# TheShadow29/VidSitu

Hardware: AMD Instinct MI355X
Metric: clips/s (10s@32x224x224) SlowFast+TxEnc fwd+bwd (higher is better)
Workload: dtype bf16

## Files before the change

### vidsitu_amd/csrc/conv_wgrad.hip

```cpp
#include <stdlib.h>

#include "common.h"

#include <mutex>
#include <type_traits>
#include "glue_bodies.h"

typedef __attribute__((ext_vector_type(4))) short s16x4;
typedef __attribute__((address_space(3))) s16x4 lds_s16x4;

struct WgradP {
  const uint16_t* dy;
  const uint16_t* x;
  float* out;
  int P;
  int Cout, Kp, Cin, x_ld, dy_ld;
  int To, Ho, Wo, Ti, Hi, Wi;
  int kT, kH, kW, sT, sH, sW, pT, pH, pW;
  int tilesM, tilesN, S, rows_per_split;
  unsigned x_bytes, dy_bytes;
  int xcd_order;
  int dbg;
  const float* in_scale;
  const float* in_shift;
};

#define WG_OOB 0x80000000u

#define WG_ROWTAB 1024

__device__ __forceinline__ int wg_swz_chunk(int row) {
  return ((row & 3) << 1) | (((row >> 3) & 1) << 3);
}

template <int BM, int BN, int WM, int WN, int MODE>
__global__ __launch_bounds__(256) void conv_wgrad_kernel(WgradP p) {
  extern __shared__ __attribute__((aligned(16))) char smem[];
  constexpr int TM = BM / WM, TN = BN / WN;
  constexpr int MR = TM / 16, NR = TN / 16;
  constexpr int CM = BM / 8, CN = BN / 8;
  constexpr int RPM = 256 / CM, RPN = 256 / CN;
  constexpr int IM = (64 + RPM - 1) / RPM, IN = (64 + RPN - 1) / RPN;
  constexpr int IMG = 64 * 256;
  constexpr int STAGE = 2 * IMG;
  static_assert(WM * WN == 4, "4 waves");

  const int tid = threadIdx.x;
  int bid = blockIdx.x;
  if (p.xcd_order) {
    const int nwg = gridDim.x, q = nwg >> 3, r = nwg & 7, xcd = blockIdx.x & 7;
    bid = (xcd < r ? xcd * (q + 1) : r * (q + 1) + (xcd - r) * q) + (blockIdx.x >> 3);
  }
  const int ntile = p.tilesM * p.tilesN;
  const int s = bid / ntile;
  bid -= s * ntile;
  const int tn = bid % p.tilesN, tm = bid / p.tilesN;
  const int m0 = tm * BM, n0 = tn * BN;
  const int pbeg = s * p.rows_per_split;
  const int pend = min(p.P, pbeg + p.rows_per_split);

  int4* rowtab = (int4*)(smem + 2 * STAGE);

  const int ccm = tid % CM, rm = tid / CM;
  const int ccn = tid % CN, rn = tid / CN;
  const bool mcol_ok = (m0 + ccm * 8) < p.Cout;
  const int ncol = n0 + ccn * 8;
  const bool ncol_ok = ncol < p.Kp;
  int dt = 0, dh = 0, dw = 0, c0 = 0;
  if (MODE == 1 && ncol_ok) {
    const int tap = ncol / p.Cin;
    c0 = ncol - tap * p.Cin;
    dw = tap % p.kW;
    const int t2 = tap / p.kW;
    dh = t2 % p.kH;
    dt = t2 / p.kH;
  }

  u32x4 ra[IM], rb[IN];
  const __amdgpu_buffer_rsrc_t xsrc =
      __builtin_amdgcn_make_buffer_rsrc((void*)p.x, 0, (int)p.x_bytes, 0x00020000);
  const __amdgpu_buffer_rsrc_t dysrc =
      __builtin_amdgcn_make_buffer_rsrc((void*)p.dy, 0, (int)p.dy_bytes, 0x00020000);
  const unsigned dycol = (unsigned)((m0 + ccm * 8) * 2);
  const unsigned xtap = (MODE == 1)
      ? (unsigned)(((((long long)dt * p.Hi + dh) * p.Wi + dw) * p.x_ld + c0) * 2)
      : (unsigned)(ncol * 2);

  auto gload = [&](int pstep, int chunk0) __attribute__((always_inline)) {
#pragma unroll
    for (int i = 0; i < IM; ++i) {
      const int r = rm + RPM * i;
      const int pp = pstep + r;
      const unsigned ok = (unsigned)(r < 64) & (unsigned)mcol_ok & (unsigned)(pp < pend);
      const unsigned off = ok ? (unsigned)pp * (unsigned)(p.dy_ld * 2) + dycol : WG_OOB;
      ra[i] = __builtin_bit_cast(u32x4, __builtin_amdgcn_raw_buffer_load_b128(dysrc, off, 0, 0));
    }
#pragma unroll
    for (int i = 0; i < IN; ++i) {
      const int r = rn + RPN * i;
      const int pp = pstep + r;
      unsigned ok = (unsigned)(r < 64) & (unsigned)ncol_ok & (unsigned)(pp < pend);
      unsigned off;
      if (MODE == 0) {
        off = (unsigned)pp * (unsigned)(p.x_ld * 2) + xtap;
      } else {
        const int4 e = rowtab[(pp - chunk0) & (WG_ROWTAB - 1)];
        const int ti = e.y + dt, hi = e.z + dh, wi = e.w + dw;
        ok &= (unsigned)((unsigned)ti < (unsigned)p.Ti) & (unsigned)((unsigned)hi < (unsigned)p.Hi) &
              (unsigned)((unsigned)wi < (unsigned)p.Wi);
        off = (unsigned)e.x + xtap;
      }
      rb[i] = __builtin_bit_cast(u32x4, __builtin_amdgcn_raw_buffer_load_b128(xsrc, ok ? off : WG_OOB, 0, 0));
    }
  };

  auto sstore = [&](int buf) __attribute__((always_inline)) {
    char* A = smem + buf * STAGE;
    char* B = A + IMG;
#pragma unroll
    for (int i = 0; i < IM; ++i) {
      const int r = rm + RPM * i;
      if (r < 64) *(u32x4*)(A + r * 256 + ((ccm ^ wg_swz_chunk(r)) << 4)) = ra[i];
    }
#pragma unroll
    for (int i = 0; i < IN; ++i) {
      const int r = rn + RPN * i;
      if (r < 64) *(u32x4*)(B + r * 256 + ((ccn ^ wg_swz_chunk(r)) << 4)) = rb[i];
    }
  };

  const int wave = tid >> 6, lane = tid & 63;
  const int wm = wave / WN, wn = wave % WN;
  const int g = lane >> 4, li = lane & 15, q = li >> 2, pp4 = li & 3;

  f32x4 acc[MR][NR];
#pragma unroll
  for (int a = 0; a < MR; ++a)
#pragma unroll
    for (int b = 0; b < NR; ++b) acc[a][b] = (f32x4){0.f, 0.f, 0.f, 0.f};

  auto compute = [&](int buf) __attribute__((always_inline)) {
    const char* A = smem + buf * STAGE;
    const char* B = A + IMG;
#pragma unroll
    for (int ks = 0; ks < 2; ++ks) {
      const int row = ks * 32 + 8 * g + q;
      const int swz = ((row & 3) << 2) | (((row >> 3) & 1) << 4);
      bf16x8 af[MR], bfr[NR];
#pragma unroll
      for (int a = 0; a < MR; ++a) {
        const int unit = ((wm * TM + a * 16) >> 2) + pp4;
        const lds_s16x4* ptr = (const lds_s16x4*)(A + row * 256 + ((unit ^ swz) << 3));
        const s16x4 lo = __builtin_amdgcn_ds_read_tr16_b64_v4i16((lds_s16x4*)ptr);
        const s16x4 hi = __builtin_amdgcn_ds_read_tr16_b64_v4i16((lds_s16x4*)(ptr + 128));
        typedef __attribute__((ext_vector_type(8))) short s16x8;
        const s16x8 v = __builtin_shufflevector(lo, hi, 0, 1, 2, 3, 4, 5, 6, 7);
        af[a] = __builtin_bit_cast(bf16x8, v);
      }
#pragma unroll
      for (int b = 0; b < NR; ++b) {
        const int unit = ((wn * TN + b * 16) >> 2) + pp4;
        const lds_s16x4* ptr = (const lds_s16x4*)(B + row * 256 + ((unit ^ swz) << 3));
        const s16x4 lo = __builtin_amdgcn_ds_read_tr16_b64_v4i16((lds_s16x4*)ptr);
        const s16x4 hi = __builtin_amdgcn_ds_read_tr16_b64_v4i16((lds_s16x4*)(ptr + 128));
        typedef __attribute__((ext_vector_type(8))) short s16x8;
        const s16x8 v = __builtin_shufflevector(lo, hi, 0, 1, 2, 3, 4, 5, 6, 7);
        bfr[b] = __builtin_bit_cast(bf16x8, v);
      }
#pragma unroll
      for (int a = 0; a < MR; ++a)
#pragma unroll
        for (int b = 0; b < NR; ++b)
          acc[a][b] = __builtin_amdgcn_mfma_f32_16x16x32_bf16(af[a], bfr[b], acc[a][b], 0, 0, 0);
    }
  };

  for (int chunk0 = pbeg; chunk0 < pend; chunk0 += WG_ROWTAB) {
    const int cend = min(pend, chunk0 + WG_ROWTAB);
    if (MODE == 1) {
      __syncthreads();
      for (int i = tid; i < WG_ROWTAB; i += 256) {
        const int pp = chunk0 + i;
        int4 e = make_int4(0, -(1 << 20), -(1 << 20), -(1 << 20));
        if (pp < cend) {
          int wo, t1, ho, t2, to, n;
          if (p.P < (1 << 24)) {
            fast_divmod(pp, p.Wo, 1.0f / (float)p.Wo, t1, wo);
            fast_divmod(t1, p.Ho, 1.0f / (float)p.Ho, t2, ho);
            fast_divmod(t2, p.To, 1.0f / (float)p.To, n, to);
          } else {
            wo = pp % p.Wo; t1 = pp / p.Wo;
            ho = t1 % p.Ho; t2 = t1 / p.Ho;
            to = t2 % p.To; n = t2 / p.To;
          }
          e.y = to * p.sT - p.pT;
          e.z = ho * p.sH - p.pH;
          e.w = wo * p.sW - p.pW;
          const long long pos0 = (((long long)n * p.Ti + e.y) * p.Hi + e.z) * p.Wi + e.w;
          e.x = (int)(unsigned)(pos0 * p.x_ld * 2);
        }
        rowtab[i] = e;
      }
      __syncthreads();
    }
    const int nsteps = (cend - chunk0 + 63) >> 6;
    gload(chunk0, chunk0);
    __syncthreads();
    sstore(0);
    __syncthreads();
    for (int st = 0; st < nsteps - 1; ++st) {
      const int cur = st & 1;
      gload(chunk0 + (st + 1) * 64, chunk0);
      __builtin_amdgcn_sched_barrier(0);
      compute(cur);
      __builtin_amdgcn_sched_barrier(0);
      sstore(cur ^ 1);
      __syncthreads();
    }
    compute((nsteps - 1) & 1);
    __syncthreads();
  }

  float* dst = p.out + (long long)s * p.Cout * p.Kp;
#pragma unroll
  for (int a = 0; a < MR; ++a)
#pragma unroll
    for (int b = 0; b < NR; ++b) {
      const int col = n0 + wn * TN + b * 16 + li;
#pragma unroll
      for (int r = 0; r < 4; ++r) {
        const int row = m0 + wm * TM + a * 16 + g * 4 + r;
        if (row < p.Cout && col < p.Kp) dst[(long long)row * p.Kp + col] = acc[a][b][r];
      }
    }
}

template <int BM, int BN, int WM, int WN, int MODE, int NS, bool AOL = false, int ROWS = 64>
__device__ __forceinline__ void conv_wgrad_ring_body(const WgradP& p, const int blk, const int nblk) {
  static_assert(!AOL || MODE == 0, "apply on load: pointwise launches");
  static_assert(ROWS == 64, "stage depth (the half-depth variant of round 4 was measured slower and removed)");
  extern __shared__ __attribute__((aligned(16))) char smem[];
  constexpr int TM = BM / WM, TN = BN / WN;
  constexpr int MR = TM / 16, NR = TN / 16;
  constexpr int CM = BM / 8, CN = BN / 8;
  constexpr int IMG = ROWS * 256;
  constexpr int STAGE = 2 * IMG;
  constexpr int D = NS - 1;
  constexpr int RG = ROWS / 16;
  constexpr int L = 2 * RG;
  constexpr int SPC = WG_ROWTAB / ROWS;
  static_assert(WM * WN == 4, "4 waves");
  static_assert((D - 1) * L <= 63, "vmcnt range");

  const int tid = threadIdx.x;
  int bid = blk;
  if (p.xcd_order) {
    const int nwg = nblk, q = nwg >> 3, r = nwg & 7, xcd = blk & 7;
    bid = (xcd < r ? xcd * (q + 1) : r * (q + 1) + (xcd - r) * q) + (blk >> 3);
  }
  const int ntile = p.tilesM * p.tilesN;
  const int s = bid / ntile;
  bid -= s * ntile;
  const int tn = bid % p.tilesN, tm = bid / p.tilesN;
  const int m0 = tm * BM, n0 = tn * BN;
  const int pbeg = s * p.rows_per_split;
  const int pend = min(p.P, pbeg + p.rows_per_split);
  const int nsteps = (pend - pbeg + ROWS - 1) / ROWS;
  int2* rowtab = (int2*)(smem + NS * STAGE);

  const int wv = __builtin_amdgcn_readfirstlane(tid >> 6), lane = tid & 63;
  const int rg = lane >> 4, cc = lane & 15;
  const int lc = cc ^ ((rg << 1) | ((wv >> 1) << 3));
  const bool mcol_ok = lc < CM && (m0 + lc * 8) < p.Cout;
  const int ncol = n0 + lc * 8;
  const bool ncol_ok = lc < CN && ncol < p.Kp;
  int tap = 0, c0 = 0, dt = 0, dh = 0, dw = 0;
  if (MODE == 1 && ncol_ok) {
    tap = ncol / p.Cin;
    c0 = ncol - tap * p.Cin;
    dw = tap % p.kW;
    const int t2 = tap / p.kW;
    dh = t2 % p.kH;
    dt = t2 / p.kH;
  }
  const unsigned dycol = (unsigned)((m0 + lc * 8) * 2);
  const unsigned xtap = (MODE == 1)
      ? (unsigned)(((((long long)dt * p.Hi + dh) * p.Wi + dw) * p.x_ld + c0) * 2)
      : (unsigned)(ncol * 2);
  const unsigned dy_pitch = (unsigned)(p.dy_ld * 2), x_pitch = (unsigned)(p.x_ld * 2);

  typedef __attribute__((address_space(3))) char* lds_ptr_t;
  const unsigned lds0 = (unsigned)(unsigned long)(lds_ptr_t)smem + (unsigned)wv * 1024u;
  auto rsrc_words = [](const void* base, unsigned bytes) __attribute__((always_inline)) {
    const unsigned long a = (unsigned long)base;
    return (i32x4){(int)(unsigned)a, (int)((unsigned)(a >> 32) & 0xffffu), (int)bytes, 0x00020000};
  };
  const i32x4 xdesc = rsrc_words(p.x, p.x_bytes), dydesc = rsrc_words(p.dy, p.dy_bytes);
  auto dma16 = [](const i32x4& desc, unsigned lds_addr, unsigned voff) __attribute__((always_inline)) {
    asm volatile("s_mov_b32 m0, %0\n\ts_nop 0\n\tbuffer_load_dwordx4 %1, %2, 0 offen lds"
                 :
                 : "s"(lds_addr), "v"(voff), "s"(desc)
                 : "memory");
  };

  const bool small_p = p.P < (1 << 24);
  const float rcpWo = 1.0f / (float)p.Wo, rcpHo = 1.0f / (float)p.Ho, rcpTo = 1.0f / (float)p.To;
  auto build_tab = [&](int chunk) __attribute__((always_inline)) {
    int2* tab = rowtab + (chunk & 1) * WG_ROWTAB;
    const int base = pbeg + chunk * WG_ROWTAB;
    for (int i = tid; i < WG_ROWTAB; i += 256) {
      const int pp = base + i;
      int2 e = make_int2(0, 0);
      if (pp < pend) {
        int wo, t1, ho, t2, to, n;
        if (small_p) {
          fast_divmod(pp, p.Wo, rcpWo, t1, wo);
          fast_divmod(t1, p.Ho, rcpHo, t2, ho);
          fast_divmod(t2, p.To, rcpTo, n, to);
        } else {
          wo = pp % p.Wo; t1 = pp / p.Wo;
          ho = t1 % p.Ho; t2 = t1 / p.Ho;
          to = t2 % p.To; n = t2 / p.To;
        }
        const int ti0 = to * p.sT - p.pT, hi0 = ho * p.sH - p.pH, wi0 = wo * p.sW - p.pW;
        const long long pos0 = (((long long)n * p.Ti + ti0) * p.Hi + hi0) * p.Wi + wi0;
        e.x = (int)(unsigned)(pos0 * p.x_ld * 2);
        unsigned mt = 0u, mh = 0u, mw = 0u;
        for (int a = 0; a < p.kT; ++a) mt |= ((unsigned)(ti0 + a) < (unsigned)p.Ti ? 1u : 0u) << a;
        for (int a = 0; a < p.kH; ++a) mh |= ((unsigned)(hi0 + a) < (unsigned)p.Hi ? 1u : 0u) << a;
        for (int a = 0; a < p.kW; ++a) mw |= ((unsigned)(wi0 + a) < (unsigned)p.Wi ? 1u : 0u) << a;
        unsigned mk = 0u;
        int tp = 0;
        for (int a = 0; a < p.kT; ++a)
          for (int b = 0; b < p.kH; ++b) {
            const unsigned th = (mt >> a) & (mh >> b) & 1u;
            mk |= (th ? mw : 0u) << tp;
            tp += p.kW;
          }
        e.y = (int)mk;
      }
      tab[i] = e;
    }
  };

  auto dma = [&](int st, int stage) __attribute__((always_inline)) {
    const unsigned A = lds0 + (unsigned)(stage * STAGE);
    const unsigned B = A + IMG;
    const int rel0 = st * ROWS + 4 * wv + rg;
    int2 ent[RG];
    if (MODE == 1) {
#pragma unroll
      for (int i = 0; i < RG; ++i) {
        const int rel = rel0 + 16 * i;
        ent[i] = rowtab[((rel >> 10) & 1) * WG_ROWTAB + (rel & (WG_ROWTAB - 1))];
      }
    }
#pragma unroll
    for (int i = 0; i < RG; ++i) {
      const int rel = rel0 + 16 * i;
      const int pp = pbeg + rel;
      const unsigned ok = (unsigned)mcol_ok & (unsigned)(pp < pend);
      dma16(dydesc, A + i * 4096, ok ? (unsigned)pp * dy_pitch + dycol : WG_OOB);
    }
#pragma unroll
    for (int i = 0; i < RG; ++i) {
      const int rel = rel0 + 16 * i;
      const int pp = pbeg + rel;
      unsigned ok = (unsigned)ncol_ok & (unsigned)(pp < pend);
      unsigned off;
      if (MODE == 0) {
        off = (unsigned)pp * x_pitch + xtap;
      } else {
        ok &= ((unsigned)ent[i].y >> tap) & 1u;
        off = (unsigned)ent[i].x + xtap;
      }
      dma16(xdesc, B + i * 4096, ok ? off : WG_OOB);
    }
  };

  const int wm = wv / WN, wn = wv % WN;
  const int g = lane >> 4, li = lane & 15, q = li >> 2, pp4 = li & 3;
  f32x4 acc[MR][NR];
#pragma unroll
  for (int a = 0; a < MR; ++a)
#pragma unroll
    for (int b = 0; b < NR; ++b) acc[a][b] = (f32x4){0.f, 0.f, 0.f, 0.f};

  float asc[NR], ash[NR];
#pragma unroll
  for (int b = 0; b < NR; ++b) {
    const int col = n0 + wn * TN + b * 16 + li;
    asc[b] = (AOL && col < p.Kp) ? p.in_scale[col] : 0.f;
    ash[b] = (AOL && col < p.Kp) ? p.in_shift[col] : 0.f;
  }
  auto compute = [&](int stage) __attribute__((always_inline)) {
    const char* A = smem + stage * STAGE;
    const char* B = A + IMG;
#pragma unroll
    for (int ks = 0; ks < ROWS / 32; ++ks) {
      const int row = ks * 32 + 8 * g + q;
      const int swz = ((row & 3) << 2) | (((row >> 3) & 1) << 4);
      bf16x8 af[MR], bfr[NR];
      typedef __attribute__((ext_vector_type(8))) short s16x8;
#pragma unroll
      for (int a = 0; a < MR; ++a) {
        const int unit = ((wm * TM + a * 16) >> 2) + pp4;
        const lds_s16x4* ptr = (const lds_s16x4*)(A + row * 256 + ((unit ^ swz) << 3));
        const s16x4 lo = __builtin_amdgcn_ds_read_tr16_b64_v4i16((lds_s16x4*)ptr);
        const s16x4 hi = __builtin_amdgcn_ds_read_tr16_b64_v4i16((lds_s16x4*)(ptr + 128));
        af[a] = __builtin_bit_cast(bf16x8, (s16x8)__builtin_shufflevector(lo, hi, 0, 1, 2, 3, 4, 5, 6, 7));
      }
#pragma unroll
      for (int b = 0; b < NR; ++b) {
        const int unit = ((wn * TN + b * 16) >> 2) + pp4;
        const lds_s16x4* ptr = (const lds_s16x4*)(B + row * 256 + ((unit ^ swz) << 3));
        const s16x4 lo = __builtin_amdgcn_ds_read_tr16_b64_v4i16((lds_s16x4*)ptr);
        const s16x4 hi = __builtin_amdgcn_ds_read_tr16_b64_v4i16((lds_s16x4*)(ptr + 128));
        bfr[b] = __builtin_bit_cast(bf16x8, (s16x8)__builtin_shufflevector(lo, hi, 0, 1, 2, 3, 4, 5, 6, 7));
        if (AOL) bfr[b] = aol_frag_n(bfr[b], asc[b], ash[b]);
      }
#pragma unroll
      for (int a = 0; a < MR; ++a)
#pragma unroll
        for (int b = 0; b < NR; ++b)
          acc[a][b] = __builtin_amdgcn_mfma_f32_16x16x32_bf16(af[a], bfr[b], acc[a][b], 0, 0, 0);
    }
  };

  if (MODE == 1) {
    build_tab(0);
    __syncthreads();
  }
#pragma unroll
  for (int d = 0; d < D; ++d) dma(d, d);
  int st_c = 0, st_l = D;
  for (int st = 0; st < nsteps; ++st) {
    if (!(p.dbg & 4)) asm volatile("s_waitcnt vmcnt(%0) lgkmcnt(0)" ::"i"((D - 1) * L) : "memory");
    if (!(p.dbg & 8)) __builtin_amdgcn_s_barrier();
    __builtin_amdgcn_sched_barrier(0);
    if (MODE == 1 && (st % SPC) == 0 && pbeg + (st / SPC + 1) * WG_ROWTAB < pend && !(p.dbg & 32))
      build_tab(st / SPC + 1);
    if (!(p.dbg & 2)) dma(st + D, st_l);
    __builtin_amdgcn_sched_barrier(0);
    if (!(p.dbg & 1)) compute(st_c);
    __builtin_amdgcn_sched_barrier(0);
    st_c = (st_c + 1 == NS) ? 0 : st_c + 1;
    st_l = (st_l + 1 == NS) ? 0 : st_l + 1;
  }
  asm volatile("s_waitcnt vmcnt(0)" ::: "memory");
  if ((p.dbg & 64) && acc[0][0][0] != 123.456f) return;

  float* dst = p.out + (long long)s * p.Cout * p.Kp;
#pragma unroll
  for (int a = 0; a < MR; ++a)
#pragma unroll
    for (int b = 0; b < NR; ++b) {
      const int col = n0 + wn * TN + b * 16 + li;
#pragma unroll
      for (int r = 0; r < 4; ++r) {
        const int row = m0 + wm * TM + a * 16 + g * 4 + r;
        if (row < p.Cout && col < p.Kp) dst[(long long)row * p.Kp + col] = acc[a][b][r];
      }
    }
}

template <int BM, int BN, int WM, int WN, int MODE, int NS, bool AOL = false, int ROWS = 64>
__global__ __launch_bounds__(256) void conv_wgrad_ring_kernel(WgradP p) {
  conv_wgrad_ring_body<BM, BN, WM, WN, MODE, NS, AOL, ROWS>(p, blockIdx.x, gridDim.x);
}

#define WGD_UNIT (3 * 8192)
#define WGD_NU 6
#define WGD_TAB 512
#define WGD_EP 260

template <int MODE, bool STAG>
__device__ __forceinline__ void conv_wgrad_deep_body(const WgradP& p, const int blk, const int nblk) {
  extern __shared__ __attribute__((aligned(16))) char smem[];
  const int tid = threadIdx.x;
  const int wv = __builtin_amdgcn_readfirstlane(tid >> 6), lane = tid & 63;
  const int hf = wv >> 2, wq = wv & 3;
  int bid = blk;
  if (p.xcd_order) {
    const int nwg = nblk, q = nwg >> 3, r = nwg & 7, xcd = blk & 7;
    bid = (xcd < r ? xcd * (q + 1) : r * (q + 1) + (xcd - r) * q) + (blk >> 3);
  }
  const int ntile = p.tilesM * p.tilesN;
  const int s = bid / ntile;
  bid -= s * ntile;
  const int tn = bid % p.tilesN, tm = bid / p.tilesN;
  const int m0 = tm * 128, n0 = tn * 256;
  const int pbeg = s * p.rows_per_split;
  const int pend = min(p.P, pbeg + p.rows_per_split);
  const int nu = (pend - pbeg + 31) >> 5;
  int2* rowtab = (int2*)(smem + WGD_NU * WGD_UNIT);

  const int rg = lane >> 4, cc = lane & 15;
  const int lc = cc ^ ((rg << 1) | (((STAG ? wv : wq) >> 1 & 1) << 3));
  const bool mcol_ok = (m0 + lc * 8) < p.Cout;
  const unsigned dycol = (unsigned)((m0 + lc * 8) * 2);
  bool ncol_ok[2];
  int tap[2];
  unsigned xtap[2];
#pragma unroll
  for (int i = 0; i < 2; ++i) {
    const int ncol = n0 + i * 128 + lc * 8;
    ncol_ok[i] = ncol < p.Kp;
    tap[i] = 0;
    xtap[i] = (unsigned)(ncol * 2);
    if (MODE == 1 && ncol_ok[i]) {
      tap[i] = ncol / p.Cin;
      const int c0 = ncol - tap[i] * p.Cin;
      const int dw = tap[i] % p.kW, t2 = tap[i] / p.kW;
      const int dh = t2 % p.kH, dt = t2 / p.kH;
      xtap[i] = (unsigned)(((((long long)dt * p.Hi + dh) * p.Wi + dw) * p.x_ld + c0) * 2);
    }
  }
  const unsigned dy_pitch = (unsigned)(p.dy_ld * 2), x_pitch = (unsigned)(p.x_ld * 2);
  typedef __attribute__((address_space(3))) char* lds_ptr_t;
  const unsigned lds0 = (unsigned)(unsigned long)(lds_ptr_t)smem + (unsigned)(STAG ? wv : wq) * 1024u;
  auto rsrc_words = [](const void* base, unsigned bytes) __attribute__((always_inline)) {
    const unsigned long a = (unsigned long)base;
    return (i32x4){(int)(unsigned)a, (int)((unsigned)(a >> 32) & 0xffffu), (int)bytes, 0x00020000};
// ... 932 lines not shown
```

Before: 730.9.

## Deepen register prefetch for narrow wgrad tiles and stream the row table in halves

For narrow tiles (BM<=32) the wgrad kernel now keeps R=D-1 stages of global loads in flight in registers instead of one, so memory latency is hidden behind more compute steps. The per-chunk row-table rebuild, which stalled the pipeline behind two barriers, becomes a double-buffered half-table that is refilled while loads continue. In exchange it uses more VGPRs, which may lower occupancy, and the tail and modular indexing logic gets harder to follow. Wider tiles keep the old depth-2 path.

Measured after the change: 740.2, median of 6. 1.01x the previous value.

```diff
diff --git a/vidsitu_amd/csrc/conv_wgrad.hip b/vidsitu_amd/csrc/conv_wgrad.hip
--- a/vidsitu_amd/csrc/conv_wgrad.hip
+++ b/vidsitu_amd/csrc/conv_wgrad.hip
@@ -33,9 +33,16 @@
   return ((row & 3) << 1) | (((row >> 3) & 1) << 3);
 }
 
+#ifndef WG_NARROW_DEPTH
+#define WG_NARROW_DEPTH 3
+#endif
+constexpr int wg_depth(int bm) { return bm <= 32 ? WG_NARROW_DEPTH : 2; }
+
 template <int BM, int BN, int WM, int WN, int MODE>
 __global__ __launch_bounds__(256) void conv_wgrad_kernel(WgradP p) {
   extern __shared__ __attribute__((aligned(16))) char smem[];
+  constexpr int D = wg_depth(BM), R = D - 1;
+  static_assert(D >= 2 && R * 64 < WG_ROWTAB / 2, "loads never run past the table half being rebuilt");
   constexpr int TM = BM / WM, TN = BN / WN;
   constexpr int MR = TM / 16, NR = TN / 16;
   constexpr int CM = BM / 8, CN = BN / 8;
@@ -76,7 +83,7 @@
     dt = t2 / p.kH;
   }
 
-  u32x4 ra[IM], rb[IN];
+  u32x4 ra[R][IM], rb[R][IN];
   const __amdgpu_buffer_rsrc_t xsrc =
       __builtin_amdgcn_make_buffer_rsrc((void*)p.x, 0, (int)p.x_bytes, 0x00020000);
   const __amdgpu_buffer_rsrc_t dysrc =
@@ -86,15 +93,17 @@
       ? (unsigned)(((((long long)dt * p.Hi + dh) * p.Wi + dw) * p.x_ld + c0) * 2)
       : (unsigned)(ncol * 2);
 
-  auto gload = [&](int pstep, int chunk0) __attribute__((always_inline)) {
+  auto gload_a = [&](int u, int pstep) __attribute__((always_inline)) {
 #pragma unroll
     for (int i = 0; i < IM; ++i) {
       const int r = rm + RPM * i;
       const int pp = pstep + r;
       const unsigned ok = (unsigned)(r < 64) & (unsigned)mcol_ok & (unsigned)(pp < pend);
       const unsigned off = ok ? (unsigned)pp * (unsigned)(p.dy_ld * 2) + dycol : WG_OOB;
-      ra[i] = __builtin_bit_cast(u32x4, __builtin_amdgcn_raw_buffer_load_b128(dysrc, off, 0, 0));
-    }
+      ra[u][i] = __builtin_bit_cast(u32x4, __builtin_amdgcn_raw_buffer_load_b128(dysrc, off, 0, 0));
+    }
+  };
+  auto gload_b = [&](int u, int pstep) __attribute__((always_inline)) {
 #pragma unroll
     for (int i = 0; i < IN; ++i) {
       const int r = rn + RPN * i;
@@ -104,28 +113,53 @@
       if (MODE == 0) {
         off = (unsigned)pp * (unsigned)(p.x_ld * 2) + xtap;
       } else {
-        const int4 e = rowtab[(pp - chunk0) & (WG_ROWTAB - 1)];
+        const int4 e = rowtab[(pp - pbeg) & (WG_ROWTAB - 1)];
         const int ti = e.y + dt, hi = e.z + dh, wi = e.w + dw;
         ok &= (unsigned)((unsigned)ti < (unsigned)p.Ti) & (unsigned)((unsigned)hi < (unsigned)p.Hi) &
               (unsigned)((unsigned)wi < (unsigned)p.Wi);
         off = (unsigned)e.x + xtap;
       }
-      rb[i] = __builtin_bit_cast(u32x4, __builtin_amdgcn_raw_buffer_load_b128(xsrc, ok ? off : WG_OOB, 0, 0));
-    }
-  };
-
-  auto sstore = [&](int buf) __attribute__((always_inline)) {
+      rb[u][i] = __builtin_bit_cast(u32x4, __builtin_amdgcn_raw_buffer_load_b128(xsrc, ok ? off : WG_OOB, 0, 0));
+    }
+  };
+
+  auto sstore = [&](int u, int buf) __attribute__((always_inline)) {
     char* A = smem + buf * STAGE;
     char* B = A + IMG;
 #pragma unroll
     for (int i = 0; i < IM; ++i) {
       const int r = rm + RPM * i;
-      if (r < 64) *(u32x4*)(A + r * 256 + ((ccm ^ wg_swz_chunk(r)) << 4)) = ra[i];
+      if (r < 64) *(u32x4*)(A + r * 256 + ((ccm ^ wg_swz_chunk(r)) << 4)) = ra[u][i];
     }
 #pragma unroll
     for (int i = 0; i < IN; ++i) {
       const int r = rn + RPN * i;
-      if (r < 64) *(u32x4*)(B + r * 256 + ((ccn ^ wg_swz_chunk(r)) << 4)) = rb[i];
+      if (r < 64) *(u32x4*)(B + r * 256 + ((ccn ^ wg_swz_chunk(r)) << 4)) = rb[u][i];
+    }
+  };
+
+  auto build_tab = [&](int rel0, int count) __attribute__((always_inline)) {
+    for (int i = tid; i < count; i += 256) {
+      const int pp = pbeg + rel0 + i;
+      int4 e = make_int4(0, -(1 << 20), -(1 << 20), -(1 << 20));
+      if (pp < pend) {
+        int wo, t1, ho, t2, to, n;
+        if (p.P < (1 << 24)) {
+          fast_divmod(pp, p.Wo, 1.0f / (float)p.Wo, t1, wo);
+          fast_divmod(t1, p.Ho, 1.0f / (float)p.Ho, t2, ho);
+          fast_divmod(t2, p.To, 1.0f / (float)p.To, n, to);
+        } else {
+          wo = pp % p.Wo; t1 = pp / p.Wo;
+          ho = t1 % p.Ho; t2 = t1 / p.Ho;
+          to = t2 % p.To; n = t2 / p.To;
+        }
+        e.y = to * p.sT - p.pT;
+        e.z = ho * p.sH - p.pH;
+        e.w = wo * p.sW - p.pW;
+        const long long pos0 = (((long long)n * p.Ti + e.y) * p.Hi + e.z) * p.Wi + e.w;
+        e.x = (int)(unsigned)(pos0 * p.x_ld * 2);
+      }
+      rowtab[(rel0 + i) & (WG_ROWTAB - 1)] = e;
     }
   };
 
@@ -175,50 +209,65 @@
     }
   };
 
-  for (int chunk0 = pbeg; chunk0 < pend; chunk0 += WG_ROWTAB) {
-    const int cend = min(pend, chunk0 + WG_ROWTAB);
+  if constexpr (D == 2) {
+    for (int chunk0 = pbeg; chunk0 < pend; chunk0 += WG_ROWTAB) {
+      const int cend = min(pend, chunk0 + WG_ROWTAB);
+      if (MODE == 1) {
+        __syncthreads();
+        build_tab(chunk0 - pbeg, WG_ROWTAB);
+        __syncthreads();
+      }
+      const int nsteps = (cend - chunk0 + 63) >> 6;
+      gload_a(0, chunk0);
+      gload_b(0, chunk0);
+      __syncthreads();
+      sstore(0, 0);
+      __syncthreads();
+      for (int st = 0; st < nsteps - 1; ++st) {
+        const int cur = st & 1;
+        gload_a(0, chunk0 + (st + 1) * 64);
+        gload_b(0, chunk0 + (st + 1) * 64);
+        __builtin_amdgcn_sched_barrier(0);
+        compute(cur);
+        __builtin_amdgcn_sched_barrier(0);
+        sstore(0, cur ^ 1);
+        __syncthreads();
+      }
+      compute((nsteps - 1) & 1);
+      __syncthreads();
+    }
+  } else {
+    constexpr int HALF = WG_ROWTAB / 2, SPH = HALF / 64;
+    const int nsteps = (pend - pbeg + 63) >> 6;
+#pragma unroll
+    for (int u = 0; u < R; ++u) gload_a(u, pbeg + u * 64);
     if (MODE == 1) {
+      build_tab(0, HALF);
       __syncthreads();
-      for (int i = tid; i < WG_ROWTAB; i += 256) {
-        const int pp = chunk0 + i;
-        int4 e = make_int4(0, -(1 << 20), -(1 << 20), -(1 << 20));
-        if (pp < cend) {
-          int wo, t1, ho, t2, to, n;
-          if (p.P < (1 << 24)) {
-            fast_divmod(pp, p.Wo, 1.0f / (float)p.Wo, t1, wo);
-            fast_divmod(t1, p.Ho, 1.0f / (float)p.Ho, t2, ho);
-            fast_divmod(t2, p.To, 1.0f / (float)p.To, n, to);
-          } else {
-            wo = pp % p.Wo; t1 = pp / p.Wo;
-            ho = t1 % p.Ho; t2 = t1 / p.Ho;
-            to = t2 % p.To; n = t2 / p.To;
-          }
-          e.y = to * p.sT - p.pT;
-          e.z = ho * p.sH - p.pH;
-          e.w = wo * p.sW - p.pW;
-          const long long pos0 = (((long long)n * p.Ti + e.y) * p.Hi + e.z) * p.Wi + e.w;
-          e.x = (int)(unsigned)(pos0 * p.x_ld * 2);
-        }
-        rowtab[i] = e;
-      }
+    }
+#pragma unroll
+    for (int u = 0; u < R; ++u) gload_b(u, pbeg + u * 64);
+    sstore(0, 0);
+    __syncthreads();
+    auto iter = [&](int u, int st) __attribute__((always_inline)) {
+      if (MODE == 1 && (st & (SPH - 1)) == 0 && pbeg + (st / SPH + 1) * HALF < pend) build_tab((st / SPH + 1) * HALF, HALF);
+      gload_a(u, pbeg + (st + R) * 64);
+      gload_b(u, pbeg + (st + R) * 64);
+      __builtin_amdgcn_sched_barrier(0);
+      compute(st & 1);
+      __builtin_amdgcn_sched_barrier(0);
+      sstore((u + 1) % R, (st + 1) & 1);
       __syncthreads();
-    }
-    const int nsteps = (cend - chunk0 + 63) >> 6;
-    gload(chunk0, chunk0);
-    __syncthreads();
-    sstore(0);
-    __syncthreads();
-    for (int st = 0; st < nsteps - 1; ++st) {
-      const int cur = st & 1;
-      gload(chunk0 + (st + 1) * 64, chunk0);
-      __builtin_amdgcn_sched_barrier(0);
-      compute(cur);
-      __builtin_amdgcn_sched_barrier(0);
-      sstore(cur ^ 1);
-      __syncthreads();
-    }
-    compute((nsteps - 1) & 1);
-    __syncthreads();
+    };
+    int st = 0;
+    for (; st + R < nsteps; st += R) {
+#pragma unroll
+      for (int u = 0; u < R; ++u) iter(u, st + u);
+    }
+#pragma unroll
+    for (int u = 0; u < R - 1; ++u)
+      if (st + u < nsteps - 1) iter(u, st + u);
+    if (nsteps > 0) compute((nsteps - 1) & 1);
   }
 
   float* dst = p.out + (long long)s * p.Cout * p.Kp;
```
